# nebula-beta/MonocularSfM

Hardware: AMD Instinct MI355X
Metric: descriptor-pairs/sec (and image-pairs/sec); match-index bit-parity vs CPU (higher is better)
Workload: dtype f32

## Files before the change

### monocularsfm_amd/csrc/msfm_kernels.hip.h

```cpp
#pragma once
#include <hip/hip_runtime.h>
#include <stdint.h>
#include "msfm_hostutil.h"

#pragma clang fp contract(off)

namespace msfm {

constexpr int kDim = 128;
constexpr int kBM = 128;
constexpr int kBN = 128;
constexpr int kTM = 8;
constexpr int kTN = 4;
constexpr int kThreads = 512;
constexpr int kChunkPos = 32;
constexpr int kChunks = kDim / kChunkPos;
constexpr int kPanelFloats = kBM * kDim;
constexpr int kSlotFloats = kChunkPos * kBN;
constexpr int kWaveCols = kBN / 8;
constexpr int kWaveSlotFloats = kChunkPos * kWaveCols;
constexpr int kLdsA = 0;
constexpr int kLdsB = kPanelFloats;
constexpr int kLdsFloats = kLdsB + 8 * 2 * kWaveSlotFloats;
constexpr int kLdsBytes = kLdsFloats * 4;
// ... 440 lines not shown
        const float* other = fwd ? pd.b_rawp : pd.a_rawp;
        const int n_other = fwd ? pd.n2 : pd.n1;
        const long long ko = (fwd ? pd.kf_off : pd.kr_off) + w.z;
        const float d0 = k_d0[ko];
        int best = 0x7fffffff;
        for (int t = threadIdx.x; t < n_other; t += 64) {
            const float s = fwd ? l2sqr_rowmajor<ORDER>(me, other + (size_t)t * kDim)
                                : l2sqr_rowmajor<ORDER>(other + (size_t)t * kDim, me);
            if (sqrtf(s) == d0) { best = t; break; }
        }
#pragma unroll
        for (int m = 32; m >= 1; m >>= 1) best = min(best, __shfl_xor(best, m));
        if (threadIdx.x == 0 && best != 0x7fffffff) k_i0[ko] = best;
    }
}

struct EpiParams {
    float ratio;
    int cross_check;
    double max_distance;
};

__device__ __forceinline__ bool order_sensitive(int i0, float d0, float d1, float ratio, double max_distance, bool forward) {
    return msfm_order_sensitive(i0, d0, d1, ratio, max_distance, forward);
}
__device__ __forceinline__ bool lowe_keep(int i0, float d0, float d1, float ratio) {
    return (i0 >= 0) && (d1 < kNoNeighbour || d1 == f_inf()) && (d0 < ratio * d1);
}

struct KnnFromArrays {
    const int* i0;
    const float* d0;
    const float* d1;
    __device__ __forceinline__ void get(long long slot, bool , int& i, float& a, float& b) const {
        i = i0[slot];
        a = d0[slot];
        b = d1[slot];
    }
};
struct KnnFromKeys {
    const float* tuv;
    const unsigned long long* best;
    const unsigned long long* second;
    int cap;
    __device__ __forceinline__ void get(long long slot, bool reverse, int& i, float& a, float& b) const {
        i = -1;
        a = b = kNoNeighbour;
        if (tuv[slot] == -f_inf()) return;
        const unsigned long long kb = best[slot], ks = second[slot];
        if (kb != ~0ull) { i = (int)(unsigned)(kb & 0xffffffffu); a = sqrtf(__uint_as_float((unsigned)(kb >> 32))); }
        if (ks != ~0ull) b = sqrtf(__uint_as_float((unsigned)(ks >> 32)));
        else if (cap && reverse && kb != ~0ull) b = f_inf();
    }
};

template <class KNN>
__global__ __launch_bounds__(256) void epilogue_kernel(const PairDesc* __restrict__ pairs, EpiParams prm, KNN knn,
                                                       int2* __restrict__ st_qt, float* __restrict__ st_d,
                                                       int* __restrict__ counts, int* __restrict__ sens_counts) {
    MSFM_TAIL_PRIO();
    const PairDesc pd = pairs[blockIdx.x];
    __shared__ int wsum[4];
    __shared__ int running, n_sens;
    if (threadIdx.x == 0) { running = 0; n_sens = 0; }
    __syncthreads();
    if (!pd.valid || pd.n2 < 2 || (prm.cross_check && pd.n1 < 2)) {
        if (threadIdx.x == 0) { counts[blockIdx.x] = 0; sens_counts[blockIdx.x] = 0; }
        return;
    }
    const bool certify = !pd.exact_int;
    const int lane = threadIdx.x & 63, wave = threadIdx.x >> 6;
    for (int q0 = 0; q0 < pd.n1; q0 += 256) {
        const int q = q0 + threadIdx.x;
        bool keep = false, sens = false;
        int t = -1;
        float d0 = 0.f;
        if (q < pd.n1) {
            float d1;
            knn.get(pd.kf_off + q, false, t, d0, d1);
            keep = lowe_keep(t, d0, d1, prm.ratio);
            sens = certify && order_sensitive(t, d0, d1, prm.ratio, prm.max_distance, true);
            if (keep && prm.cross_check) {
                int rq;
                float rd0, rd1;
                knn.get(pd.kr_off + t, true, rq, rd0, rd1);
                const bool rkeep = lowe_keep(rq, rd0, rd1, prm.ratio);
                const int vis = rkeep ? rq : 0;
                keep = (vis == q);
            }
            if (keep && ((double)d0 > prm.max_distance)) keep = false;
        }
        const unsigned long long sb = __ballot(sens);
        if (lane == 0 && sb) atomicAdd(&n_sens, __popcll(sb));
        const unsigned long long bal = __ballot(keep);
        const int before = __popcll(bal & ((1ull << lane) - 1ull));
        if (lane == 0) wsum[wave] = __popcll(bal);
        __syncthreads();
        int off = running;
        for (int w = 0; w < wave; ++w) off += wsum[w];
        if (keep) {
            st_qt[pd.out_off + off + before] = make_int2(q, t);
            st_d[pd.out_off + off + before] = d0;
        }
        __syncthreads();
        if (threadIdx.x == 0) running += wsum[0] + wsum[1] + wsum[2] + wsum[3];
        __syncthreads();
    }
    if (certify && prm.cross_check)
        for (int t0 = 0; t0 < pd.n2; t0 += 256) {
            const int t = t0 + threadIdx.x;
            int ri = -1;
            float rd0 = 0.f, rd1 = 0.f;
            if (t < pd.n2) knn.get(pd.kr_off + t, true, ri, rd0, rd1);
            const bool s = t < pd.n2 && order_sensitive(ri, rd0, rd1, prm.ratio, prm.max_distance, false);
            const unsigned long long sb = __ballot(s);
            if (lane == 0 && sb) atomicAdd(&n_sens, __popcll(sb));
        }
    __syncthreads();
    if (threadIdx.x == 0) { counts[blockIdx.x] = running; sens_counts[blockIdx.x] = n_sens; }
}

__global__ void scan_counts_kernel(const int* __restrict__ counts, long long* __restrict__ offsets, int n) {
    MSFM_TAIL_PRIO();
    __shared__ long long carry;
    __shared__ long long wtot[4];
    if (threadIdx.x == 0) carry = 0;
    __syncthreads();
    const int lane = threadIdx.x & 63, wave = threadIdx.x >> 6;
    for (int base = 0; base < n; base += 256) {
        const int i = base + threadIdx.x;
        long long v = (i < n) ? counts[i] : 0;
        long long incl = v;
#pragma unroll
        for (int m = 1; m < 64; m <<= 1) {
            const long long o = __shfl_up(incl, m);
            if (lane >= m) incl += o;
        }
        if (lane == 63) wtot[wave] = incl;
        __syncthreads();
        long long woff = carry;
        for (int w = 0; w < wave; ++w) woff += wtot[w];
        if (i < n) offsets[i] = woff + incl - v;
        __syncthreads();
        if (threadIdx.x == 0) carry += wtot[0] + wtot[1] + wtot[2] + wtot[3];
        __syncthreads();
    }
    if (threadIdx.x == 0) offsets[n] = carry;
}

// ... 16 lines not shown
```

### monocularsfm_amd/csrc/msfm_batch.hip.h

```cpp
#pragma once
namespace {
struct Batch {
    std::vector<PairDesc> pairs;
    std::vector<PfPair> pf;
    std::vector<int> id1, id2;
    std::vector<int> item_base;
    size_t n_items = 0, items_per_xcd = 0;
    MsfmItemChunks chunks = {};
    long long rp_elems = 0, cp_elems = 0, kf_elems = 0, kr_elems = 0, out_elems = 0, cand_elems = 0;
    int max_npad = 0;
    int64_t desc_pairs = 0;
    int64_t algo_bytes = 0;
    MsfmRoute route;
    std::vector<CandList> dense_lists;
    std::vector<VerifyPair> verify_pairs;
};

void build_items(Batch& b, int path, const std::vector<char>* only = nullptr, std::vector<int>* base_out = nullptr,
                 MsfmItemChunks* chunks_out = nullptr, const std::vector<char>* idle = nullptr) {
    std::vector<int> order(b.pairs.size());
    for (size_t p = 0; p < order.size(); ++p) order[p] = (int)p;
    if (b.id2.size() == b.pairs.size())
        std::stable_sort(order.begin(), order.end(), [&](int x, int y) { return b.id2[(size_t)x] < b.id2[(size_t)y]; });
    std::vector<int>& base = base_out ? *base_out : b.item_base;
// ... 477 lines not shown
    HIPCHK(ctx, SC.d_tu.ensure(kn * 4));
    HIPCHK(ctx, SC.d_colmask.ensure(kn * 4));
    HIPCHK(ctx, SC.d_best.ensure(kn * 8));
    HIPCHK(ctx, SC.d_second.ensure(kn * 8));
    HIPCHK(ctx, SC.d_overflow.ensure(P));
    HIPCHK(ctx, SC.d_totals.ensure(kTotalsBytes));
    FillBatch fills;
    if (!route.compact()) {
        fills.add(SC.d_best.p, (size_t)kn * 8, 0xff);
        fills.add(SC.d_second.p, (size_t)kn * 8, 0xff);
    }
    fills.add(SC.d_totals.p, kTotalsBytes, 0);
    fills.add(SC.d_overflow.p, P, 0);
    const int rc = upload_pair_tables(ctx, b, 1, route.q8() ? &pfq : nullptr, fills, route.kind == kRouteQ8Mixed ? &pf16 : nullptr,
                                        route.kind == kRouteQ8Mixed ? &item_base16 : nullptr, route.kind == kRouteQ8Mixed ? &chunks16 : nullptr);
    if (rc != MSFM_OK) return rc;
    return MSFM_OK;
    }

    int launch_sweep1() {
        e0 = get_event(ctx, ev_base), e1 = get_event(ctx, ev_base + 1);
        e2 = get_event(ctx, ev_base + 2), e3 = get_event(ctx, ev_base + 3);
        if (!e0 || !e1 || !e2 || !e3) return fail(ctx, MSFM_E_DEVICE, "hipEventCreate failed");
        block = dim3(kPfThreads);
        sweep_grid = (unsigned)std::max(8, (ctx->cu_count / 8) * 8);
        dp = SC.d_pairs.as<PairDesc>();
        dpf = SC.d_pf.as<PfPair>();
        tuv = SC.d_tu.as<float>();
        colmask = SC.d_colmask.as<unsigned>();
        hc.lap("sweep-1 setup + uploads");
        if (ctx->last_sweep1 && ctx->last_sweep1 != ctx->cur)
            HIPCHK(ctx, hipStreamWaitEvent(SC.stream, ctx->last_sweep1->sweep1_done, 0));
        for (Scratch& other : ctx->sc)
            if (&other != ctx->cur && other.sweep2_recorded && other.seq + 2 <= SC.seq)
                HIPCHK(ctx, hipStreamWaitEvent(SC.stream, other.sweep2_done, 0));
        unsigned long long* wg_end = nullptr;
        if (ctx->wg_trace && (route.kind == kRouteI8 || route.q8())) {
            HIPCHK(ctx, SC.d_wg_end.ensure((size_t)sweep_grid * 16));
            wg_end = SC.d_wg_end.as<unsigned long long>();
            SC.pf_pending.wg_trace_grid = (int)std::min<unsigned>(sweep_grid, (unsigned)b.n_items);
        }
        int* cursors = SC.d_totals.as<int>() + kTotalsSweep1;
        HIPCHK(ctx, hipEventRecord(e0, SC.stream));
        if (route.kind == kRouteI8 || route.q8())
            hipLaunchKernelGGL(sweep_i8_kernel<1>, dim3(std::min<unsigned>(sweep_grid, (unsigned)b.n_items)), dim3(kI8Threads), kI8LdsBytes1, SC.stream, dp,
                               route.q8() ? (const PfPair*)SC.d_pfq.as<PfPair>() : dpf,
                               SC.d_items.as<WorkItem>(), SC.d_rp_s0.as<float>(), SC.d_rp_s1.as<float>(), SC.d_cp_s0.as<float>(),
                               (const float*)nullptr, (int2*)nullptr, (unsigned long long*)nullptr, (const int*)nullptr, (int)b.n_items, cursors, b.chunks,
                               (int*)nullptr, wg_end);
        else
            hipLaunchKernelGGL(sweep_kernel<1>, dim3(std::min<unsigned>(sweep_grid, (unsigned)b.n_items)), block, kPfLdsBytes, SC.stream, dp, dpf,
                               SC.d_items.as<WorkItem>(), SC.d_rp_s0.as<float>(), SC.d_rp_s1.as<float>(),
                               SC.d_cp_s0.as<float>(), (float*)nullptr, (const float*)nullptr, (const float*)nullptr,
                               (int2*)nullptr, (unsigned long long*)nullptr, (const int*)nullptr, (int)b.n_items, cursors, b.chunks);
        HIPCHK(ctx, hipGetLastError());
        if (route.kind == kRouteQ8Mixed && per16) {
            hipLaunchKernelGGL(sweep_kernel<1>, dim3(std::min<unsigned>(sweep_grid, (unsigned)(per16 * 8))), block, kPfLdsBytes, SC.stream, dp,
                               (const PfPair*)SC.d_pf16.as<PfPair>(), SC.d_items16.as<WorkItem>(), SC.d_rp_s0.as<float>(), SC.d_rp_s1.as<float>(),
                               SC.d_cp_s0.as<float>(), (float*)nullptr, (const float*)nullptr, (const float*)nullptr,
                               (int2*)nullptr, (unsigned long long*)nullptr, (const int*)nullptr, (int)(per16 * 8), SC.d_totals.as<int>() + kTotalsSweep1b, chunks16);
            HIPCHK(ctx, hipGetLastError());
            SC.prof.mixed_route_sub_batches += 1;
    }
    DBGSYNC(ctx, "sweep_kernel<1>");
    HIPCHK(ctx, hipEventRecord(e1, SC.stream));
    HIPCHK(ctx, hipEventRecord(SC.sweep1_done, SC.stream));
    SC.sweep1_recorded = true;
// ... 250 lines not shown
            else if (ctx->order == MSFM_ORDER_AVX2_FMA) MSFM_LAUNCH_EXACT(1);
            else MSFM_LAUNCH_EXACT(3);
#undef MSFM_LAUNCH_EXACT
            HIPCHK(ctx, hipGetLastError());
            DBGSYNC(ctx, "pf_exact_candidates_kernel");
    }
    if (!SC.keys_epilogue) {
        hipLaunchKernelGGL(pf_finalize_kernel, mgrid, dim3(256), 0, SC.stream, dp, dpf, (const float*)tuv, SC.d_best.as<unsigned long long>(),
                           SC.d_second.as<unsigned long long>(), SC.d_k_i0.as<int>(), SC.d_k_d0.as<float>(),
                           SC.d_k_d1.as<float>(), SC.d_fix_count.as<int>(), SC.d_fix_list.as<int4>(), SC.fix_cap_eff, prune.cap);
        HIPCHK(ctx, hipGetLastError());
        DBGSYNC(ctx, "pf_finalize_kernel");
    }
    if (n_lists > 0) {
        hipLaunchKernelGGL(pf_overflow_kernel, dim3((unsigned)((n_lists + 255) / 256)), dim3(256), 0, SC.stream, dl, (int)n_lists,
                           (const unsigned long long*)SC.d_cand_count.as<unsigned long long>(), (const PlanGroup*)SC.d_groups.as<PlanGroup>(),
                           (const int*)SC.d_gmembers.as<int>(), (const int*)SC.d_member_pair.as<int>(),
                           SC.d_overflow.as<unsigned char>(), SC.d_totals.as<unsigned long long>());
        HIPCHK(ctx, hipGetLastError());
    }
    SC.pf_pending.active = true;
    SC.pf_pending.n_lists = n_lists;
    SC.pf_pending.P = P;
    SC.pf_pending.ev_base = ev_base;
    hc.lap("launch sweep 2 .. finalize");
    return MSFM_OK;
    }

    int run() {
        int rc = apply_route();
        if (rc != MSFM_OK) return rc;
        rc = build_and_upload();
        if (rc != MSFM_OK || b.n_items == 0) return rc;
        rc = launch_sweep1();
        if (rc != MSFM_OK) return rc;
        if (route.compact()) {
            rc = plan_buffers();
            if (rc == MSFM_OK && route.q8()) rc = launch_route_q();
            if (rc == MSFM_OK) rc = launch_compact_sweep2();
        } else {
            rc = launch_dense_sweep2();
        }
        if (rc != MSFM_OK) return rc;
        return launch_exact_and_finalize();
    }
};

int run_prefilter(msfm_ctx* ctx, Batch& b, size_t ev_base, PruneParams prune) {
    PrefilterLaunch launch(ctx, b, ev_base, prune);
    return launch.run();
}

int finish_prefilter(msfm_ctx* ctx, Batch& b, std::vector<char>& force_exact, bool* retry) {
    *retry = false;
    PfPending& pe = SC.pf_pending;
    if (!pe.active) return MSFM_OK;
    pe.active = false;
    const char* hs = SC.h_summary.as<char>();
    PlanSummary sm = {};
    unsigned long long totals[2] = {0, 0};
    std::memcpy(totals, hs + kHsTotals, 16);
    float ms = 0.f;
    HIPCHK(ctx, hipEventElapsedTime(&ms, ctx->ev_pool[pe.ev_base], ctx->ev_pool[pe.ev_base + 1]));
    SC.prof.approx_kernel_ms += ms;
    HIPCHK(ctx, hipEventElapsedTime(&ms, ctx->ev_pool[pe.ev_base + 2], ctx->ev_pool[pe.ev_base + 3]));
    SC.prof.sweep2_ms += ms;
    if (pe.wg_trace_grid > 0) {
        std::vector<unsigned long long> st((size_t)pe.wg_trace_grid * 2);
        HIPCHK(ctx, hipMemcpy(st.data(), SC.d_wg_end.p, st.size() * 8, hipMemcpyDeviceToHost));
        unsigned long long t0 = ~0ull, t1 = 0;
// ... 232 lines not shown
```

### monocularsfm_amd/csrc/msfm_ctx.hip.h

```cpp
#pragma once
namespace {

struct AllocClock {
    double dev_ms = 0, pin_ms = 0, free_ms = 0;
    long long dev_bytes = 0, pin_bytes = 0;
    int dev_n = 0, pin_n = 0, free_n = 0;
    static double now() { return std::chrono::duration<double, std::milli>(std::chrono::steady_clock::now().time_since_epoch()).count(); }
};
inline AllocClock& alloc_clock() {
    static thread_local AllocClock c;
    return c;
}
inline hipError_t timed_malloc(void** p, size_t bytes) {
    const double t0 = AllocClock::now();
    const hipError_t e = hipMalloc(p, bytes);
    AllocClock& c = alloc_clock();
    c.dev_ms += AllocClock::now() - t0;
    c.dev_bytes += (long long)bytes;
    c.dev_n += 1;
    return e;
}
inline void timed_free(void* p) {
    const double t0 = AllocClock::now();
    (void)hipFree(p);
// ... 388 lines not shown
    void free_chunk(int i) {
        StoreChunk& c = chunks[(size_t)i];
        if (c.base) (void)hipFree(c.base);
        c = StoreChunk{};
        if (cur == i) cur = -1;
    }
    void drop(int& chunk) {
        if (chunk < 0) return;
        StoreChunk& c = chunks[(size_t)chunk];
        if (--c.live <= 0) {
            if (chunk == cur || recycle) c.used = 0, c.live = 0;
            else free_chunk(chunk);
        }
        chunk = -1;
    }
    size_t bytes() const {
        size_t s = 0;
        for (const StoreChunk& c : chunks) s += c.cap;
        return s;
    }
    void release_all() {
        for (size_t i = 0; i < chunks.size(); ++i) free_chunk((int)i);
        chunks.clear();
        cur = -1;
    }
};

constexpr int kSlots = 2 * MSFM_MAX_IMAGES + 2;
constexpr long long kDefaultScratchBytes = (long long)64 << 30;
constexpr int kDefaultMaxPairsPerBatch = 16384;
constexpr int kMaxPairsPerBatchLimit = 65535;
constexpr int kDefaultPipeline = 2;
constexpr double kDefaultTaper = 1.0;
constexpr int kInFlight = 3;
constexpr long long kMinPipelineCost = 15000000000LL;

}

struct PfPending {
    bool active = false, compact = false, refine = false;
    size_t n_lists = 0, P = 0;
    long long rows_cap = 0, cand_cap = 0, items_cap = 0;
    long long rows_ub = 0;
    int compact_pairs = 0;
    long long dense_swept = 0;
    size_t ev_base = 0;
    int wg_trace_grid = 0;
};

struct Scratch {
    hipStream_t stream = nullptr;
    DevBuf d_up[3];
    PinnedBuf h_up[3];
    Ref d_pairs, d_pf, d_pfq, d_pf16, d_item_base, d_item_base16;
    Ref d_groups, d_gmembers, d_member_pair, d_member_group, d_ppair;
    DevBuf d_items;
    DevBuf d_rp_s0, d_rp_i0, d_rp_s1, d_cp_s0, d_cp_i0, d_cp_s1;
    DevBuf d_k_i0, d_k_d0, d_k_d1;
    DevBuf d_st_qt, d_st_d, d_counts, d_offsets, d_sens;
    DevBuf d_sub_qt, d_sub_d;
    PinnedBuf h_sub_qt, h_sub_d;
    DevBuf d_fix_count, d_fix_list;
    int fix_cap_eff = 0;
    bool keys_epilogue = false;
    DevBuf d_tu, d_tv, d_cand, d_cand_count, d_best, d_second;
    DevBuf d_cmp_tu, d_live_idx, d_row_pair, d_row_src, d_vpairs, d_vpf, d_vitems, d_lists, d_items16;
    DevBuf d_cmp_s0, d_cmp_s1, d_summary_a;
// ... 113 lines not shown

    Scratch sc[kInFlight];
    Scratch* cur = &sc[0];
    Scratch* last_sweep1 = nullptr;
    DevBuf d_zero_row;
    StoreArena store;
    StoreArena inbox;
    std::vector<int> pending;
    size_t inbox_waiting = 0;
    bool store_async = false;
    PinnedBuf up_ring;
    CopyHelper copier;
    bool copy_helper = true;
    hipEvent_t up_ev[2] = {nullptr, nullptr};
    bool up_ev_recorded[2] = {false, false};
    unsigned up_seq = 0;
    DevBuf d_jobs, d_store_maxima;
    PinnedBuf h_jobs, h_store_maxima;
    PinnedPool pinned_pool;
    hipEvent_t jobs_ev = nullptr;
    size_t store_peak_bytes = 0;
    std::vector<OutSeg> out_segs;
    size_t out_used = 0;
    int fix_cap = 1 << 16;
    int max_pairs_per_batch = kDefaultMaxPairsPerBatch;
    long long scratch_bytes = 0;
    int last_hip_error = 0;
    long long budget_cached = 0;
    size_t budget_for_store = 0;
    long long budget_for_limit = 0;
    long long issue_seq = 0;
    double pipeline_taper = kDefaultTaper;
    int in_flight = kInFlight;
    bool wg_trace = false;
    int pipeline = kDefaultPipeline;
    int prefilter = 1;
    int byte_detect = 1;
    float q8_level = 0.f;
    int q8_direct = 1;
    int q8_route = 1;
    MsfmRouteKnobs route_knobs() const { return MsfmRouteKnobs{prefilter, q8_route, q8_direct, q8_level}; }
    DeferredFrees deferred;
    long long cmp_rows_hint = 0;
    long long hint_rows_ub = 0;
    long long items_hint = 0, cand_hint = 0;

    bool have_results = false;
    std::vector<int64_t> res_offsets;
    std::vector<int32_t> res_sens;
    GrowPinned res_qt, res_dist;
    size_t res_count = 0;

    msfm_profile prof = {};
    std::vector<hipEvent_t> ev_pool;
    MatchJob* job = nullptr;
    bool series_open = false;
    DevBuf ret_words, ret_cn;
    int ret_v = 0;
    msfm_retrieval_profile ret_prof = {};
    int verify_model = MSFM_VERIFY_FUNDAMENTAL;
    msfm_emat::Camera camera = {};
    long long staged_solved = 0;
    int staged_rounds = 0;
    bool model_select = false;
    double h_ratio = 0.7;
    std::vector<int32_t> sel_records;
// ... 70 lines not shown
```

### monocularsfm_amd/csrc/msfm_hostutil.h

```cpp
#pragma once
#include <cmath>
#include <vector>

#if defined(__HIPCC__)
#include <hip/hip_runtime.h>
#define MSFM_HD __host__ __device__ inline __attribute__((always_inline))
#else
#define MSFM_HD inline
#endif

MSFM_HD int msfm_cp_pack(int hi, bool hi_valid, int lo, bool lo_valid) {
    unsigned c = 255u;
    if (lo_valid) {
        const unsigned x = (unsigned)(hi - lo) + 16u;
        int e = 27 - __builtin_clz(x);
        unsigned m = (x + (1u << e) - 1u) >> e;
        e += (int)(m >> 5);
        m = (m >> 5) ? 16u : m;
        const unsigned code = ((unsigned)e << 4) | (m - 16u);
        c = code >= 255u ? 255u : code;
    }
    return hi_valid ? (int)(((unsigned)hi << 8) | c) : (int)0x80000000;
}
constexpr int kCpNone = -(1 << 23);
MSFM_HD int msfm_cp_hi(int code) { return code >> 8; }
MSFM_HD bool msfm_cp_has_second(int code) { return (code & 255) != 255; }
MSFM_HD int msfm_cp_gap(int code) { const int c = code & 255; return ((16 + (c & 15)) << (c >> 4)) - 16; }

inline std::vector<long long> msfm_pipeline_marks(long long total, long long n_sub, double taper) {
    std::vector<long long> marks;
    if (n_sub < 2) return marks;
    const double last = taper, first = 2.0 - last;
    double acc = 0.0;
    marks.push_back(0);
    for (long long k = 0; k < n_sub; ++k) {
        acc += first - (first - last) * (double)k / (double)(n_sub - 1);
        marks.push_back(k + 1 == n_sub ? total : (long long)((double)total * acc / (double)n_sub));
    }
    return marks;
}

constexpr int kItemChunks = 8;
struct MsfmItemChunks {
    int start[kItemChunks + 1];
    int items() const { return start[kItemChunks]; }
    int longest() const {
        int m = 0;
        for (int x = 0; x < kItemChunks; ++x) m = start[x + 1] - start[x] > m ? start[x + 1] - start[x] : m;
        return m;
    }
};
MSFM_HD int msfm_item_chunk_of(const MsfmItemChunks& c, int k) {
    int x = 0;
#pragma unroll
    for (int j = 1; j < kItemChunks; ++j) x += k >= c.start[j] ? 1 : 0;
    return x;
}
MSFM_HD long long msfm_item_position(const MsfmItemChunks& c, int k) {
    const int x = msfm_item_chunk_of(c, k);
    return (long long)(k - c.start[x]) * kItemChunks + x;
}

constexpr int kItemCostTileFixed = 16, kItemCostTileWaves = 48, kItemCostFixed = 160;
inline long long msfm_item_cost(int b_tiles, int rows, int wave_rows, int waves) {
    const int active = rows <= 0 ? 0 : (rows >= wave_rows * waves ? waves : (rows + wave_rows - 1) / wave_rows);
    const int per_simd = (active + 3) / 4, full = (waves + 3) / 4;
    return kItemCostFixed + (long long)b_tiles * (kItemCostTileFixed + kItemCostTileWaves * per_simd / full);
}

struct MsfmItemRun { long long count, cost; };
inline MsfmItemChunks msfm_item_chunks(const std::vector<MsfmItemRun>& runs) {
    MsfmItemChunks c = {};
// ... 235 lines not shown
```

### monocularsfm_amd/csrc/msfm_job.hip.h

```cpp
#pragma once

static int call_prologue(msfm_ctx* ctx) {
    HIPCHK(ctx, hipSetDevice(ctx->device));
    ctx->cur = &ctx->sc[0];
    for (Scratch& s : ctx->sc) forget_sweeps(ctx, s);
    if (!ctx->deferred.empty()) {
        HIPCHK(ctx, hipDeviceSynchronize());
        ctx->deferred.flush();
    }
    return settle_store(ctx);
}

template <class Attempt>
static int rerun_alone(msfm_ctx* ctx, Attempt attempt) {
    for (int k = 1;; ++k) {
        bool retry = false;
        const int rc = attempt(&retry);
        if (rc != MSFM_OK || !retry) return rc;
        if (k >= 6) return fail(ctx, MSFM_E_DEVICE, "batch kept overflowing its queues");
    }
}

struct MatchJob {
    msfm_ctx* ctx = nullptr;
    std::vector<int32_t> pairs_own;
    const int32_t* pairs = nullptr;
    int n_pairs = 0;
    msfm_match_params prm = {0.8f, 1, 0.7};
    PruneParams prune = {1, 0.8f, 0.7f};
    msfm_verify_params verify_store = {};
    const msfm_verify_params* verify = nullptr;
    bool streaming = false;
    bool select = false;
    bool pose = false;
    hipEvent_t ev_begin = nullptr, ev_end = nullptr;
    int kSets = kInFlight;
    long long kScratchBytes = 1;
    MsfmRouteKnobs knobs = {};
    int kMaxPairsPerBatch = kDefaultMaxPairsPerBatch;
    std::vector<long long> marks;
    long long cost_done = 0;
    bool need_fix = false;
    SubBatch sb[kInFlight];
    int next_begin = 0;
    long long issued = 0, completed = 0;
    bool memory_wait = false;
    int memory_shrinks = 0;

    int start(msfm_ctx* c, const int32_t* pairs_in, int n, const msfm_match_params* params, const msfm_verify_params* vp, bool stream_mode) {
        ctx = c;
        pairs = pairs_in;
        n_pairs = n;
        streaming = stream_mode;
        verify = nullptr;
        c->have_results = c->sel_valid = c->tv_valid = false;
        select = vp && c->model_select && c->verify_model != MSFM_VERIFY_HOMOGRAPHY;
        c->sel_records.assign(select && !stream_mode ? 3 * (size_t)n : 0, 0);
        pose = vp && c->two_view && c->verify_model == MSFM_VERIFY_ESSENTIAL;
        c->tv_records.assign(pose && !stream_mode ? (size_t)n : 0, msfm_two_view_record{});
        if (vp) {
            verify_store = *vp;
            verify = &verify_store;
            c->staged_solved = 0;
            c->staged_rounds = 0;
        }
        for (SubBatch& w : sb) w = SubBatch{};
        next_begin = 0;
        issued = completed = 0;
        memory_wait = false;
// ... 1 lines not shown
        ctx->last_hip_error = 0;
        prm = msfm_match_params{0.8f, 1, 0.7};
        if (params) prm = *params;
        prune = PruneParams{1, prm.ratio, (float)prm.max_distance};
        if ((double)prune.max_distance < prm.max_distance) prune.max_distance = nextafterf(prune.max_distance, __builtin_huge_valf());
        if (!(prm.ratio > 0.f) || !(prm.ratio <= 1.f)) prune.ratio = 0.f;
        if (!(prm.max_distance >= 0.0)) prune.max_distance = __builtin_huge_valf();
        int rc = call_prologue(ctx);
        if (rc != MSFM_OK) return rc;
        rc = rebuild_stale_twins(ctx, pairs, 2 * n_pairs);
        if (rc != MSFM_OK) return rc;
        ctx->res_offsets.assign((size_t)n_pairs + 1, 0);
        ctx->res_sens.assign((size_t)n_pairs, 0);
        ctx->res_count = 0;
        ctx->prof = msfm_profile{};
        ctx->out_used = 0;
        for (OutSeg& s : ctx->out_segs) s.count = 0;
        if (!streaming) {
            long long bound = 1;
            for (int k = 0; k < n_pairs; ++k) {
                const int i = pairs[2 * k], j = pairs[2 * k + 1];
                if (i < 0 || i >= kSlots || j < 0 || j >= kSlots) return fail(ctx, MSFM_E_INVALID, "image id out of range");
                const long long n1 = ctx->images[(size_t)i].n, n2 = ctx->images[(size_t)j].n;
                if (n1 > 0 && n2 > 0) bound += prm.cross_check ? std::min(n1, n2) : n1;
            }
            if (ctx->res_qt.reserve((size_t)bound * 8) != hipSuccess || ctx->res_dist.reserve((size_t)bound * 4) != hipSuccess)
                return fail(ctx, MSFM_E_DEVICE, "cannot reserve address space for the result lists");
        }

        ev_begin = get_event(ctx, 0), ev_end = get_event(ctx, 1);
        if (!ev_begin || !ev_end) return fail(ctx, MSFM_E_DEVICE, "hipEventCreate failed");
        HIPCHK(ctx, hipEventRecord(ev_begin, ctx->sc[0].stream));

        kSets = ctx->in_flight;
        long long budget = ctx->scratch_bytes > 0 ? ctx->scratch_bytes : kDefaultScratchBytes;
        if (ctx->budget_cached > 0 && ctx->budget_for_store == ctx->store.bytes() && ctx->budget_for_limit == ctx->scratch_bytes) {
            budget = ctx->budget_cached;
        } else {
            size_t free_b = 0, total_b = 0;
            if (hipMemGetInfo(&free_b, &total_b) == hipSuccess) {
                long long held = 0;
                for (Scratch& sc : ctx->sc) held += sc.device_bytes();
                const long long avail = (long long)free_b + held;
                budget = std::min(budget, ctx->scratch_bytes > 0 ? avail / 2 : avail / 4);
            }
            ctx->budget_cached = budget;
            ctx->budget_for_store = ctx->store.bytes();
            ctx->budget_for_limit = ctx->scratch_bytes;
        }
        kScratchBytes = std::max<long long>(1, budget / kSets);
        knobs = ctx->route_knobs();
        kMaxPairsPerBatch = ctx->max_pairs_per_batch;
        marks.clear();
        if (ctx->pipeline > 1 && n_pairs > 1) {
            long long total = 0;
            for (int k = 0; k < n_pairs; ++k) {
                const int i = pairs[2 * k], j = pairs[2 * k + 1];
                if (i < 0 || i >= kSlots || j < 0 || j >= kSlots) return fail(ctx, MSFM_E_INVALID, "image id out of range");
                const long long n1 = ctx->images[i].n, n2 = ctx->images[j].n;
                if (n1 > 0 && n2 > 0) total += n1 * n2;
            }
            marks = msfm_pipeline_marks(total, std::min<long long>(ctx->pipeline, total / kMinPipelineCost), ctx->pipeline_taper);
        }
        cost_done = 0;
        need_fix = !(prm.ratio <= 1.f);
        if (streaming) ctx->series_open = true;
        return MSFM_OK;
    }

    int build(SubBatch& w, int begin, const std::vector<char>& force_exact) {
        w.b = Batch{};
        w.begin = begin;
        if (begin == 0) cost_done = 0;
        const long long cost_begin = (begin == w.begin_of_cost) ? w.cost_begin : cost_done;
        w.begin_of_cost = begin;
        w.cost_begin = cost_begin;
        long long mark = 0;
        if (!marks.empty()) {
            size_t i = 0;
            while (i + 2 < marks.size() && cost_begin >= (marks[i] + marks[i + 1]) / 2) ++i;
            mark = marks[i + 1];
        }
        long long est = 0, cost = 0;
        int end = begin;
        while (end < n_pairs && (end - begin) < kMaxPairsPerBatch) {
            PairDesc pd;
            PfPair pp;
            int rc = fill_pair(ctx, pairs[2 * end], pairs[2 * end + 1], pd, pp);
            if (rc != MSFM_OK) return rc;
            const Image &ia = ctx->images[pairs[2 * end]], &ib = ctx->images[pairs[2 * end + 1]];
            if (verify && (ia.nk < ia.n || ib.nk < ib.n))
                return fail(ctx, MSFM_E_STATE, "geometric verification needs msfm_upload_keypoints for image " +
                                                   std::to_string(ia.nk < ia.n ? pairs[2 * end] : pairs[2 * end + 1]));
            const int route = msfm_scratch_route(knobs, prune.prune, prune.ratio, pp.use != 0, ia.is_u8, ib.is_u8);
            const long long need = pd.valid ? msfm_pair_scratch_bytes(pd.n1, pd.n2, pd.n1pad, pd.n2pad, pd.a_blocks, pd.a_blocks256, route, pose) : 0;
            const long long c = pd.valid ? (long long)pd.n1 * pd.n2 : 0;
// ... 353 lines not shown
        forget_sweeps(ctx, sc);
        ctx->last_hip_error = 0;
        memory_wait = true;
    }
    int shrink_memory() {
        int rc = drain_streams(ctx);
        if (rc != MSFM_OK) return rc;
        ctx->deferred.flush();
        for (Scratch& sc : ctx->sc) sc.release_device();
        size_t free_b = 0, total_b = 0;
        long long share = kScratchBytes / 2;
        if (hipMemGetInfo(&free_b, &total_b) == hipSuccess) share = std::min<long long>(share, (long long)(free_b / (2 * (size_t)kSets)));
        kScratchBytes = std::max<long long>(1, share);
        ctx->budget_cached = kScratchBytes * kSets;
        ctx->hint_rows_ub = 0;
        memory_wait = false;
        memory_shrinks += 1;
        ctx->prof.memory_shrinks += 1;
        if (std::getenv("MSFM_DEBUG_TIMING"))
            std::fprintf(stderr, "[msfm alloc] out of device memory: scratch given back, %.2f GiB per sub-batch from pair %d on (%zu MiB free)\n",
                         kScratchBytes / 1073741824.0, next_begin, free_b >> 20);
        return MSFM_OK;
    }

    int step(int* slot_out) {
        const DeferFreesScope defer(&ctx->deferred);
        const std::vector<char> no_force;
        while (true) {
            while (!memory_wait && next_begin < n_pairs && issued - completed < kSets) {
                const int slot = (int)(issued % kSets);
                int rc = ensure_scratch_set(ctx, slot);
                if (rc != MSFM_OK) return rc;
                ctx->cur = &ctx->sc[slot];
                rc = build(sb[slot], next_begin, no_force);
                if (rc == MSFM_OK) rc = issue(sb[slot], 2 + 12 * (size_t)slot);
                if (out_of_memory(rc)) {
                    drop_attempt(slot);
                    break;
                }
                if (rc != MSFM_OK) return rc;
                next_begin = sb[slot].end;
                ++issued;
            }
            if (issued > completed) break;
            if (!memory_wait) break;
            const int rc = shrink_memory();
            if (rc != MSFM_OK) return rc;
        }
        if (issued == completed) return fail(ctx, MSFM_E_STATE, "step() without work");
        const int slot = (int)(completed % kSets);
        ctx->cur = &ctx->sc[slot];
        std::vector<char> force_exact;
        bool retry = false;
        int rc = complete(sb[slot], force_exact, &retry);
        if (rc != MSFM_OK) return rc;
        if (retry) {
            rc = drain_streams(ctx);
            if (rc != MSFM_OK) return rc;
            ctx->deferred.flush();
            for (int k = 0; k < kSets; ++k)
                if (k != slot) forget_sweeps(ctx, ctx->sc[k]);
            ctx->last_sweep1 = nullptr;
            rc = rerun_alone(ctx, [&](bool* again) {
                int r = build(sb[slot], sb[slot].begin, force_exact);
                if (r == MSFM_OK) r = issue(sb[slot], 2 + 12 * (size_t)slot);
                return r != MSFM_OK ? r : complete(sb[slot], force_exact, again);
// ... 30 lines not shown
```

### monocularsfm_amd/csrc/msfm_match.hip

```cpp
#include "msfm_match.h"
#include "msfm_hostutil.h"
#include "msfm_guard.h"
#include "msfm_tracks.h"
#include "msfm_kernels.hip.h"
#include "msfm_prefilter.hip.h"
#include "msfm_verify.hip.h"
#include "msfm_verify_e.hip.h"
#include "msfm_verify_h.hip.h"
#include "msfm_verify_select.hip.h"
#include "msfm_verify_pose.hip.h"
#include "msfm_retrieval.hip.h"

#include <sys/mman.h>

#include <algorithm>
#include <atomic>
#include <chrono>
#include <condition_variable>
#include <mutex>
#include <thread>
#include <cstdio>
#include <cstdlib>
#include <cmath>
#include <cstring>
// ... 97 lines not shown
    ctx->job = new_match_job();
    for (Scratch& sc : ctx->sc) {
        for (PinnedBuf& h : sc.h_up) h.pool = &ctx->pinned_pool;
        sc.h_summary.pool = sc.h_tail.pool = sc.h_tk_pairs.pool = &ctx->pinned_pool;
    }
    ctx->h_jobs.pool = ctx->h_store_maxima.pool = &ctx->pinned_pool;
    ctx->cu_count = prop.multiProcessorCount;
    ctx->clock_mhz = prop.clockRate / 1000;
    std::snprintf(ctx->dev_name, sizeof(ctx->dev_name), "%s (%s)", prop.name, prop.gcnArchName);
    if (create_rest(ctx) != MSFM_OK) {
        std::fprintf(stderr, "%s\n", ctx->err.c_str());
        destroy_streams(ctx);
        ctx->d_zero_row.release();
        delete_match_job(ctx->job);
        delete ctx;
        return MSFM_E_DEVICE;
    }
    hc.lap("create: streams, events, kernel attributes, zero row");
    if (const char* e = std::getenv("MSFM_PREFILTER")) ctx->prefilter = e[0] == '2' ? 2 : (e[0] != '0');
    if (const char* e = std::getenv("MSFM_MAX_PAIRS_PER_BATCH"))
        if (std::atoi(e) > 0) ctx->max_pairs_per_batch = std::min(std::atoi(e), kMaxPairsPerBatchLimit);
    if (const char* e = std::getenv("MSFM_PIPELINE_TAPER")) {
        const double t = std::atof(e);
        if (t >= 0.05 && t <= 1.0) ctx->pipeline_taper = t;
    }
    if (const char* e = std::getenv("MSFM_BYTE_DETECT")) ctx->byte_detect = e[0] != '0';
    if (const char* e = std::getenv("MSFM_UPLOAD_THREADS")) ctx->copy_helper = std::atoi(e) != 1;
    if (const char* e = std::getenv("MSFM_Q8_DIRECT")) ctx->q8_direct = e[0] == '2' ? 2 : (e[0] != '0');
    if (const char* e = std::getenv("MSFM_Q8")) ctx->q8_route = e[0] == '2' ? 2 : (e[0] != '0');
    if (const char* e = std::getenv("MSFM_IN_FLIGHT"))
        if (std::atoi(e) >= 1 && std::atoi(e) <= kInFlight) ctx->in_flight = std::atoi(e);
    if (const char* e = std::getenv("MSFM_PIPELINE"))
        if (std::atoi(e) > 0) ctx->pipeline = std::min(std::atoi(e), 64);
#ifdef MSFM_WG_TRACE
    if (const char* e = std::getenv("MSFM_WG_TRACE")) ctx->wg_trace = e[0] != '0';
#endif
    if (const char* e = std::getenv("MSFM_SCRATCH_MIB"))
        if (std::atoll(e) > 0) ctx->scratch_bytes = std::atoll(e) * (1LL << 20);
    *out_ctx = ctx;
    return MSFM_OK;
    MSFM_API_END
}

static void destroy_streams(msfm_ctx* ctx) {
    for (Scratch& sc : ctx->sc) {
        if (sc.sweep1_done) (void)hipEventDestroy(sc.sweep1_done);
        if (sc.sweep2_done) (void)hipEventDestroy(sc.sweep2_done);
        sc.sweep2_done = nullptr;
        if (sc.stream) (void)hipStreamDestroy(sc.stream);
        sc.sweep1_done = nullptr;
        sc.stream = nullptr;
    }
}

void msfm_destroy(msfm_ctx* ctx) {
    if (!ctx) return;
    try {
    HostClock hc;
    (void)hipSetDevice(ctx->device);
    for (Scratch& sc : ctx->sc)
        if (sc.stream) (void)hipStreamSynchronize(sc.stream);
    ctx->deferred.flush();
    ctx->tracks.release();
    ctx->store.release_all();
    ctx->inbox.release_all();
    hc.lap("destroy: store");
// ... 847 lines not shown
```

Before: 6291 billion.

## Batch epilogue kernel over four rows per thread with split load/decode

Splits the KNN accessors into separate load and decode steps so each thread can issue loads for four query rows at once before decoding, raising memory-level parallelism in the epilogue. It also cuts the per-256-row barrier count from three to one by double-buffering the per-wave counts in shared memory and having every thread track the running offset in a register. The cost is more registers per thread and clamped indices that trigger redundant loads on tail rows. Cross-check gathers are also batched, with non-kept rows pointed at index 0.

Result: no change. 6281 billion (median of 2 runs) (-0.2%).

```diff
diff --git a/monocularsfm_amd/csrc/msfm_kernels.hip.h b/monocularsfm_amd/csrc/msfm_kernels.hip.h
--- a/monocularsfm_amd/csrc/msfm_kernels.hip.h
+++ b/monocularsfm_amd/csrc/msfm_kernels.hip.h
@@ -496,10 +496,12 @@
     const int* i0;
     const float* d0;
     const float* d1;
-    __device__ __forceinline__ void get(long long slot, bool , int& i, float& a, float& b) const {
-        i = i0[slot];
-        a = d0[slot];
-        b = d1[slot];
+    struct Raw { int i; float a, b; };
+    __device__ __forceinline__ Raw load(long long slot) const { return Raw{i0[slot], d0[slot], d1[slot]}; }
+    __device__ __forceinline__ void decode(const Raw& r, bool , int& i, float& a, float& b) const {
+        i = r.i;
+        a = r.a;
+        b = r.b;
     }
 };
 struct KnnFromKeys {
@@ -507,26 +509,30 @@
     const unsigned long long* best;
     const unsigned long long* second;
     int cap;
-    __device__ __forceinline__ void get(long long slot, bool reverse, int& i, float& a, float& b) const {
+    struct Raw { float t; unsigned long long kb, ks; };
+    __device__ __forceinline__ Raw load(long long slot) const { return Raw{tuv[slot], best[slot], second[slot]}; }
+    __device__ __forceinline__ void decode(const Raw& r, bool reverse, int& i, float& a, float& b) const {
         i = -1;
         a = b = kNoNeighbour;
-        if (tuv[slot] == -f_inf()) return;
-        const unsigned long long kb = best[slot], ks = second[slot];
+        if (r.t == -f_inf()) return;
+        const unsigned long long kb = r.kb, ks = r.ks;
         if (kb != ~0ull) { i = (int)(unsigned)(kb & 0xffffffffu); a = sqrtf(__uint_as_float((unsigned)(kb >> 32))); }
         if (ks != ~0ull) b = sqrtf(__uint_as_float((unsigned)(ks >> 32)));
         else if (cap && reverse && kb != ~0ull) b = f_inf();
     }
 };
 
+constexpr int kEpiRows = 4;
+constexpr int kEpiPass = 256 * kEpiRows;
 template <class KNN>
 __global__ __launch_bounds__(256) void epilogue_kernel(const PairDesc* __restrict__ pairs, EpiParams prm, KNN knn,
                                                        int2* __restrict__ st_qt, float* __restrict__ st_d,
                                                        int* __restrict__ counts, int* __restrict__ sens_counts) {
     MSFM_TAIL_PRIO();
     const PairDesc pd = pairs[blockIdx.x];
-    __shared__ int wsum[4];
-    __shared__ int running, n_sens;
-    if (threadIdx.x == 0) { running = 0; n_sens = 0; }
+    __shared__ int wsum[2][kEpiRows][4];
+    __shared__ int n_sens;
+    if (threadIdx.x == 0) n_sens = 0;
     __syncthreads();
     if (!pd.valid || pd.n2 < 2 || (prm.cross_check && pd.n1 < 2)) {
         if (threadIdx.x == 0) { counts[blockIdx.x] = 0; sens_counts[blockIdx.x] = 0; }
@@ -534,51 +540,74 @@
     }
     const bool certify = !pd.exact_int;
     const int lane = threadIdx.x & 63, wave = threadIdx.x >> 6;
-    for (int q0 = 0; q0 < pd.n1; q0 += 256) {
-        const int q = q0 + threadIdx.x;
-        bool keep = false, sens = false;
-        int t = -1;
-        float d0 = 0.f;
-        if (q < pd.n1) {
+    int running = 0;
+    for (int q0 = 0, pass = 0; q0 < pd.n1; q0 += kEpiPass, pass ^= 1) {
+        typename KNN::Raw raw[kEpiRows];
+#pragma unroll
+        for (int j = 0; j < kEpiRows; ++j) raw[j] = knn.load(pd.kf_off + min(q0 + j * 256 + (int)threadIdx.x, pd.n1 - 1));
+        bool keep[kEpiRows];
+        int t[kEpiRows], sens = 0;
+        float d0[kEpiRows];
+#pragma unroll
+        for (int j = 0; j < kEpiRows; ++j) {
             float d1;
-            knn.get(pd.kf_off + q, false, t, d0, d1);
-            keep = lowe_keep(t, d0, d1, prm.ratio);
-            sens = certify && order_sensitive(t, d0, d1, prm.ratio, prm.max_distance, true);
-            if (keep && prm.cross_check) {
+            knn.decode(raw[j], false, t[j], d0[j], d1);
+            const bool in = q0 + j * 256 + (int)threadIdx.x < pd.n1;
+            keep[j] = in && lowe_keep(t[j], d0[j], d1, prm.ratio);
+            sens |= (in && certify && order_sensitive(t[j], d0[j], d1, prm.ratio, prm.max_distance, true)) ? 1 << j : 0;
+        }
+        if (prm.cross_check) {
+#pragma unroll
+            for (int j = 0; j < kEpiRows; ++j) raw[j] = knn.load(pd.kr_off + (keep[j] ? t[j] : 0));
+#pragma unroll
+            for (int j = 0; j < kEpiRows; ++j) {
                 int rq;
                 float rd0, rd1;
-                knn.get(pd.kr_off + t, true, rq, rd0, rd1);
+                knn.decode(raw[j], true, rq, rd0, rd1);
                 const bool rkeep = lowe_keep(rq, rd0, rd1, prm.ratio);
                 const int vis = rkeep ? rq : 0;
-                keep = (vis == q);
-            }
-            if (keep && ((double)d0 > prm.max_distance)) keep = false;
-        }
-        const unsigned long long sb = __ballot(sens);
-        if (lane == 0 && sb) atomicAdd(&n_sens, __popcll(sb));
-        const unsigned long long bal = __ballot(keep);
-        const int before = __popcll(bal & ((1ull << lane) - 1ull));
-        if (lane == 0) wsum[wave] = __popcll(bal);
+                keep[j] = keep[j] && vis == q0 + j * 256 + (int)threadIdx.x;
+            }
+        }
+        int before[kEpiRows];
+#pragma unroll
+        for (int j = 0; j < kEpiRows; ++j) {
+            if ((double)d0[j] > prm.max_distance) keep[j] = false;
+            const unsigned long long sb = __ballot((sens >> j) & 1);
+            if (lane == 0 && sb) atomicAdd(&n_sens, __popcll(sb));
+            const unsigned long long bal = __ballot(keep[j]);
+            before[j] = __popcll(bal & ((1ull << lane) - 1ull));
+            if (lane == 0) wsum[pass][j][wave] = __popcll(bal);
+        }
         __syncthreads();
-        int off = running;
-        for (int w = 0; w < wave; ++w) off += wsum[w];
-        if (keep) {
-            st_qt[pd.out_off + off + before] = make_int2(q, t);
-            st_d[pd.out_off + off + before] = d0;
-        }
-        __syncthreads();
-        if (threadIdx.x == 0) running += wsum[0] + wsum[1] + wsum[2] + wsum[3];
-        __syncthreads();
+#pragma unroll
+        for (int j = 0; j < kEpiRows; ++j) {
+            int off = running;
+            for (int w = 0; w < 4; ++w) {
+                const int c = wsum[pass][j][w];
+                if (w < wave) off += c;
+                running += c;
+            }
+            if (keep[j]) {
+                st_qt[pd.out_off + off + before[j]] = make_int2(q0 + j * 256 + (int)threadIdx.x, t[j]);
+                st_d[pd.out_off + off + before[j]] = d0[j];
+            }
+        }
     }
     if (certify && prm.cross_check)
-        for (int t0 = 0; t0 < pd.n2; t0 += 256) {
-            const int t = t0 + threadIdx.x;
-            int ri = -1;
-            float rd0 = 0.f, rd1 = 0.f;
-            if (t < pd.n2) knn.get(pd.kr_off + t, true, ri, rd0, rd1);
-            const bool s = t < pd.n2 && order_sensitive(ri, rd0, rd1, prm.ratio, prm.max_distance, false);
-            const unsigned long long sb = __ballot(s);
-            if (lane == 0 && sb) atomicAdd(&n_sens, __popcll(sb));
+        for (int t0 = 0; t0 < pd.n2; t0 += kEpiPass) {
+            typename KNN::Raw raw[kEpiRows];
+#pragma unroll
+            for (int j = 0; j < kEpiRows; ++j) raw[j] = knn.load(pd.kr_off + min(t0 + j * 256 + (int)threadIdx.x, pd.n2 - 1));
+#pragma unroll
+            for (int j = 0; j < kEpiRows; ++j) {
+                int ri;
+                float rd0, rd1;
+                knn.decode(raw[j], true, ri, rd0, rd1);
+                const bool s = t0 + j * 256 + (int)threadIdx.x < pd.n2 && order_sensitive(ri, rd0, rd1, prm.ratio, prm.max_distance, false);
+                const unsigned long long sb = __ballot(s);
+                if (lane == 0 && sb) atomicAdd(&n_sens, __popcll(sb));
+            }
         }
     __syncthreads();
     if (threadIdx.x == 0) { counts[blockIdx.x] = running; sens_counts[blockIdx.x] = n_sens; }
```

## Drop cross-set sweep2 gating for short pipelines and plan buffers before sweep1

Applied to the files above, without the earlier changes.

Adds a tail schedule that estimates per-pair scratch from a sample of pairs and picks the number of pipeline parts and scratch sets. When every part fits in its own in-flight set, the sweep1 wait on older sets' sweep2 completion is skipped for the first kSets batches. In that case buffer planning also moves ahead of the sweep1 launch so host work overlaps the device. In-flight capacity rises to four sets, which splits the scratch budget more ways when that many sets are used. The gated default set count stays at three.

Measured after the change: 6132 billion before, 6114 billion after. Within noise of the previous version (-0.3%).

```diff
diff --git a/monocularsfm_amd/csrc/msfm_batch.hip.h b/monocularsfm_amd/csrc/msfm_batch.hip.h
--- a/monocularsfm_amd/csrc/msfm_batch.hip.h
+++ b/monocularsfm_amd/csrc/msfm_batch.hip.h
@@ -533,7 +533,7 @@
         if (ctx->last_sweep1 && ctx->last_sweep1 != ctx->cur)
             HIPCHK(ctx, hipStreamWaitEvent(SC.stream, ctx->last_sweep1->sweep1_done, 0));
         for (Scratch& other : ctx->sc)
-            if (&other != ctx->cur && other.sweep2_recorded && other.seq + 2 <= SC.seq)
+            if (ctx->tail_gate && &other != ctx->cur && other.sweep2_recorded && other.seq + 2 <= SC.seq)
                 HIPCHK(ctx, hipStreamWaitEvent(SC.stream, other.sweep2_done, 0));
         unsigned long long* wg_end = nullptr;
         if (ctx->wg_trace && (route.kind == kRouteI8 || route.q8())) {
@@ -850,10 +850,15 @@
         if (rc != MSFM_OK) return rc;
         rc = build_and_upload();
         if (rc != MSFM_OK || b.n_items == 0) return rc;
+        const bool plan_first = route.compact() && !ctx->tail_gate && ctx->last_sweep1 && ctx->last_sweep1 != ctx->cur;
+        if (plan_first) {
+            rc = plan_buffers();
+            if (rc != MSFM_OK) return rc;
+        }
         rc = launch_sweep1();
         if (rc != MSFM_OK) return rc;
         if (route.compact()) {
-            rc = plan_buffers();
+            if (!plan_first) rc = plan_buffers();
             if (rc == MSFM_OK && route.q8()) rc = launch_route_q();
             if (rc == MSFM_OK) rc = launch_compact_sweep2();
         } else {
diff --git a/monocularsfm_amd/csrc/msfm_ctx.hip.h b/monocularsfm_amd/csrc/msfm_ctx.hip.h
--- a/monocularsfm_amd/csrc/msfm_ctx.hip.h
+++ b/monocularsfm_amd/csrc/msfm_ctx.hip.h
@@ -444,7 +444,8 @@
 constexpr int kMaxPairsPerBatchLimit = 65535;
 constexpr int kDefaultPipeline = 2;
 constexpr double kDefaultTaper = 1.0;
-constexpr int kInFlight = 3;
+constexpr int kInFlight = 4;
+constexpr int kGatedSets = 3;
 constexpr long long kMinPipelineCost = 15000000000LL;
 
 }
@@ -624,6 +625,8 @@
     long long issue_seq = 0;
     double pipeline_taper = kDefaultTaper;
     int in_flight = kInFlight;
+    bool force_gate = false;
+    bool tail_gate = true;
     bool wg_trace = false;
     int pipeline = kDefaultPipeline;
     int prefilter = 1;
diff --git a/monocularsfm_amd/csrc/msfm_hostutil.h b/monocularsfm_amd/csrc/msfm_hostutil.h
--- a/monocularsfm_amd/csrc/msfm_hostutil.h
+++ b/monocularsfm_amd/csrc/msfm_hostutil.h
@@ -38,6 +38,22 @@
         marks.push_back(k + 1 == n_sub ? total : (long long)((double)total * acc / (double)n_sub));
     }
     return marks;
+}
+
+struct MsfmTailSchedule { int parts, sets; bool gate; };
+inline MsfmTailSchedule msfm_tail_schedule(long long total_cost, long long min_cost, int pipeline, int in_flight, int gated_sets,
+                                           long long forced_parts, bool force_gate) {
+    MsfmTailSchedule s = {1, 1, true};
+    in_flight = in_flight < 1 ? 1 : in_flight;
+    gated_sets = gated_sets < 1 ? 1 : (gated_sets > in_flight ? in_flight : gated_sets);
+    const long long by_cost = min_cost > 0 ? total_cost / min_cost : pipeline;
+    const long long parts = pipeline < by_cost ? pipeline : by_cost;
+    s.parts = parts < 2 ? 1 : (int)parts;
+    const long long most = forced_parts > s.parts ? forced_parts : s.parts;
+    const bool fits = most <= in_flight;
+    s.sets = fits && most > gated_sets ? (int)most : gated_sets;
+    s.gate = force_gate || !fits;
+    return s;
 }
 
 constexpr int kItemChunks = 8;
diff --git a/monocularsfm_amd/csrc/msfm_job.hip.h b/monocularsfm_amd/csrc/msfm_job.hip.h
--- a/monocularsfm_amd/csrc/msfm_job.hip.h
+++ b/monocularsfm_amd/csrc/msfm_job.hip.h
@@ -3,6 +3,7 @@
 static int call_prologue(msfm_ctx* ctx) {
     HIPCHK(ctx, hipSetDevice(ctx->device));
     ctx->cur = &ctx->sc[0];
+    ctx->tail_gate = true;
     for (Scratch& s : ctx->sc) forget_sweeps(ctx, s);
     if (!ctx->deferred.empty()) {
         HIPCHK(ctx, hipDeviceSynchronize());
@@ -34,7 +35,8 @@
     bool select = false;
     bool pose = false;
     hipEvent_t ev_begin = nullptr, ev_end = nullptr;
-    int kSets = kInFlight;
+    int kSets = kGatedSets;
+    MsfmTailSchedule sched = {1, kGatedSets, true};
     long long kScratchBytes = 1;
     MsfmRouteKnobs knobs = {};
     int kMaxPairsPerBatch = kDefaultMaxPairsPerBatch;
@@ -102,7 +104,6 @@
         if (!ev_begin || !ev_end) return fail(ctx, MSFM_E_DEVICE, "hipEventCreate failed");
         HIPCHK(ctx, hipEventRecord(ev_begin, ctx->sc[0].stream));
 
-        kSets = ctx->in_flight;
         long long budget = ctx->scratch_bytes > 0 ? ctx->scratch_bytes : kDefaultScratchBytes;
         if (ctx->budget_cached > 0 && ctx->budget_for_store == ctx->store.bytes() && ctx->budget_for_limit == ctx->scratch_bytes) {
             budget = ctx->budget_cached;
@@ -118,9 +119,10 @@
             ctx->budget_for_store = ctx->store.bytes();
             ctx->budget_for_limit = ctx->scratch_bytes;
         }
-        kScratchBytes = std::max<long long>(1, budget / kSets);
         knobs = ctx->route_knobs();
         kMaxPairsPerBatch = ctx->max_pairs_per_batch;
+        const int gated_sets = std::min(kGatedSets, ctx->in_flight);
+        sched = MsfmTailSchedule{1, gated_sets, true};
         marks.clear();
         if (ctx->pipeline > 1 && n_pairs > 1) {
             long long total = 0;
@@ -130,8 +132,22 @@
                 const long long n1 = ctx->images[i].n, n2 = ctx->images[j].n;
                 if (n1 > 0 && n2 > 0) total += n1 * n2;
             }
-            marks = msfm_pipeline_marks(total, std::min<long long>(ctx->pipeline, total / kMinPipelineCost), ctx->pipeline_taper);
-        }
+            const int stride = std::max(1, n_pairs / 256);
+            long long scratch = 0, sampled = 0;
+            for (int k = 0; k < n_pairs; k += stride, ++sampled) {
+                const Image &ia = ctx->images[pairs[2 * k]], &ib = ctx->images[pairs[2 * k + 1]];
+                if (ia.n <= 0 || ib.n <= 0) continue;
+                const int route = msfm_scratch_route(knobs, prune.prune, prune.ratio, ctx->prefilter && ia.pf_safe && ib.pf_safe, ia.is_u8, ib.is_u8);
+                scratch += msfm_pair_scratch_bytes(ia.n, ib.n, ia.nalloc * kBM, ib.nalloc * kBN, ia.nblk, ia.nalloc * kBM / kPfWgRows, route, pose);
+            }
+            scratch = (long long)((double)scratch * (double)n_pairs / (double)std::max<long long>(1, sampled));
+            const long long share = std::max<long long>(1, budget / ctx->in_flight);
+            const long long forced = std::max((scratch + scratch / 4 + share - 1) / share, ((long long)n_pairs + kMaxPairsPerBatch - 1) / kMaxPairsPerBatch);
+            sched = msfm_tail_schedule(total, kMinPipelineCost, ctx->pipeline, ctx->in_flight, kGatedSets, forced, ctx->force_gate);
+            marks = msfm_pipeline_marks(total, sched.parts, ctx->pipeline_taper);
+        }
+        kSets = sched.sets;
+        kScratchBytes = std::max<long long>(1, budget / kSets);
         cost_done = 0;
         need_fix = !(prm.ratio <= 1.f);
         if (streaming) ctx->series_open = true;
@@ -551,6 +567,7 @@
                 int rc = ensure_scratch_set(ctx, slot);
                 if (rc != MSFM_OK) return rc;
                 ctx->cur = &ctx->sc[slot];
+                ctx->tail_gate = sched.gate || issued >= kSets;
                 rc = build(sb[slot], next_begin, no_force);
                 if (rc == MSFM_OK) rc = issue(sb[slot], 2 + 12 * (size_t)slot);
                 if (out_of_memory(rc)) {
diff --git a/monocularsfm_amd/csrc/msfm_match.hip b/monocularsfm_amd/csrc/msfm_match.hip
--- a/monocularsfm_amd/csrc/msfm_match.hip
+++ b/monocularsfm_amd/csrc/msfm_match.hip
@@ -153,6 +153,7 @@
         if (std::atoi(e) >= 1 && std::atoi(e) <= kInFlight) ctx->in_flight = std::atoi(e);
     if (const char* e = std::getenv("MSFM_PIPELINE"))
         if (std::atoi(e) > 0) ctx->pipeline = std::min(std::atoi(e), 64);
+    if (const char* e = std::getenv("MSFM_TAIL_GATE")) ctx->force_gate = e[0] == '1';
 #ifdef MSFM_WG_TRACE
     if (const char* e = std::getenv("MSFM_WG_TRACE")) ctx->wg_trace = e[0] != '0';
 #endif
```
